# Corleno/Nonstationary_Multivariate_Gaussian_Process

Hardware: AMD Instinct MI355X
Metric: log-posterior evals/sec (N=2048, D=3 nonseparable GP) (higher is better)
Workload: dtype f64

## Files before the change

### nonstationary_multivariate_gaussian_process_amd/csrc/nmgp_api.hip

```cpp
#include <cstdarg>

#include "nmgp_internal.h"

using namespace nmgpk;

enum {
    SC_LOGDET = 0,
    SC_QUAD = 1,
    SC_PRIORQ = 2,
    SC_TRACE = 40,
    SC_OUT = 48,
    SC_MISC = 56,
    SC_COUNT = 128
};

int nmgp_fail(nmgp_ctx* ctx, int code, const char* fmt, ...) {
    char buf[1024];
    va_list ap;
    va_start(ap, fmt);
    vsnprintf(buf, sizeof(buf), fmt, ap);
    va_end(ap);
    if (ctx) ctx->err = buf;
    return code;
}
// ... 774 lines not shown
    return 0;
}

static bool schur_selected(const nmgp_ctx* c, int want_grad) {
    if (want_grad || c->M < 2 || c->svc_schur == 0) return false;
    return true;
}

static int svc_batch_value_schur(nmgp_ctx* c, const double* xs, int xstride, const double* ys, long long ystride, int cps) {
    const int N = c->N, M = c->M, B = c->batch, n1 = (M - 1) * N;
    const long long P = c->P_svc;
    const int xpad = (N + 1) & 1, xoffA = N + 1 + xpad;
    const int ldA = (int)nmgp_ld((size_t)2 * N + 2), ldP = (int)nmgp_ld((size_t)n1 + 1);
    auto r64 = [](size_t v) { return (v + 63) / 64 * 64; };
    const size_t offP = r64((size_t)ldA * N), offPart = r64(offP + (size_t)ldP * n1);
    const size_t need = offPart + (size_t)N * ((N + 255) / 256);
    const size_t bsS = nmgp_ld((size_t)c->n + 1) * (size_t)c->n;
    double* base = c->b_S;
    size_t bsz = bsS;
    if (need > bsS) {
        if (c->b_schur_stride != need) {
            NMGP_TRY(nmgp_dev_alloc(c, &c->b_schur, (size_t)B * need));
            c->b_schur_stride = need;
        }
        base = c->b_schur;
        bsz = need;
    }
    const long long bs = (long long)bsz;
    double* A = base;
    double* Sp = base + offP;
    double* part = base + offPart;
    double* w = c->b_z;
    double* w1 = c->b_z + (size_t)B * N;
    const double* tse = c->b_pars + (P - 1);
    hipStream_t s = c->stream;
    HIP_TRY(c, hipMemsetAsync(c->b_info2, 0, (size_t)B * sizeof(int), s));
    {
        StageScope sp(c, NMGP_STAGE_COV);
        svc_prep(s, c->b_pars, N, M, c->b_ell, c->b_Lv, B);
        int r = svc_schur_build(s, 0, xs, c->b_ell, c->b_Lv, tse, ys, A, ldA, nullptr, nullptr, 0, N, M, B, bs, xstride, ystride, cps);
        if (r) return nmgp_fail(c, r, "unsupported number of outputs M=%d", M);
    }
    {
        StageScope sp(c, NMGP_STAGE_CHOL);
        identity_rows(s, A, ldA, N + 1, N, xpad, B, bs);
        potrf_lower(s, c->stream2, nmgp_chol_events(c, N), A, ldA, N, 1 + xpad, N, c->chol_nb1, c->b_info, B, bs, 1,
                    nmgp_syrk_hook(c));
    }
    {
        StageScope sp(c, NMGP_STAGE_SOLVE);
        get_row(s, A, ldA, N, w, N, B, bs, N);
        tri_gemv_upper(s, A + xoffA, ldA, N, w, c->b_u, part, B, bs, bs);
    }
    {
        StageScope sp(c, NMGP_STAGE_REDUCE);
        chol_logdet_quad(s, A, ldA, N, w, c->b_scal + 2, c->b_scal + 3, B, bs, 16);
    }
    {
        StageScope sp(c, NMGP_STAGE_INVERSE);
        syrk_lower(s, A + xoffA, ldA, A, ldA, N, N, N, B, bs, bs, 2);
    }
    {
        StageScope sp(c, NMGP_STAGE_COV);
        int r = svc_schur_build(s, 1, xs, c->b_ell, c->b_Lv, tse, ys, A, ldA, c->b_u, Sp, ldP, N, M, B, bs, xstride, ystride, cps);
        if (r) return nmgp_fail(c, r, "unsupported number of outputs M=%d", M);
    }
    {
        StageScope sp(c, NMGP_STAGE_CHOL);
        potrf_lower(s, c->stream2, nmgp_chol_events(c, n1), Sp, ldP, n1, 1, 0, c->chol_nb1, c->b_info2, B, bs, 1,
                    nmgp_syrk_hook(c));
    }
    {
        StageScope sp(c, NMGP_STAGE_SOLVE);
        get_row(s, Sp, ldP, n1, w1, n1, B, bs, n1);
    }
    {
        StageScope sp(c, NMGP_STAGE_REDUCE);
        chol_logdet_quad(s, Sp, ldP, n1, w1, c->b_scal + 4, c->b_scal + 5, B, bs, 16);
        svc_schur_combine(s, c->b_Lv, N, M, c->b_scal, 16, c->b_info, c->b_info2, B);
// ... 879 lines not shown
```

### nonstationary_multivariate_gaussian_process_amd/csrc/nmgp_chol.hip

```cpp
#include "nmgp_internal.h"
#include <cstring>

namespace nmgpk {

static inline int cdiv_c(long long a, long long b) { return (int)((a + b - 1) / b); }

typedef double v4d __attribute__((ext_vector_type(4)));

#define SY_BM 128
#define SY_BK 16
#define SY_LD (SY_BM + 16)
#define SY_SB 8

__device__ __forceinline__ int clamp_row_pair(int r, int rows) {
    int rc = r < rows - 1 ? r : rows - 2;
    return rc < 0 ? 0 : rc;
}

__device__ __forceinline__ double fast_recip(double p) {
    double x = __builtin_amdgcn_rcp(p);
    double e = fma(-p, x, 1.0);
    x = fma(x, e, x);
    e = fma(-p, x, 1.0);
    x = fma(x, e, x);
// ... 67 lines not shown
#undef PF
    __syncthreads();
#pragma unroll
    for (int kk = 0; kk < 16; ++kk) {
        const int c = 4 * kk + g;
        if (r < nb && c <= r) A[(size_t)c * lda + r] = a[kk] * rsqrt(pivs[c]);
    }
}

typedef double v2d __attribute__((ext_vector_type(2)));
typedef int v4i __attribute__((ext_vector_type(4)));

__device__ __forceinline__ void syrk_fused_first_block(double* lds, const v4d (&acc)[2][2][2], bool owner, int wj,
                                                       double* __restrict__ C, int ldc, int* __restrict__ info, int goff);

__device__ __forceinline__ void syrk_tile_fast(const double* __restrict__ A, int lda, double* __restrict__ C, int ldc, int K,
                                               int row0, int col0, bool diag, int kt0, bool beta0, int ncw, int yrow,
                                               int nyr, double* sA0, double* sB0, bool skip00 = false,
                                               int* __restrict__ finfo = nullptr, int fgoff = 0, bool mirror = false,
                                               int fresh0 = 0x7fffffff) {
    constexpr int BK = 16;
    constexpr int SBUF = BK * SY_LD;
    const int tid = threadIdx.x, lane = tid & 63, w = tid >> 6;
    const int wi = w & 1, wj = w >> 1;
    const int l15 = lane & 15, l4 = lane >> 4;
    const int rp = tid & 63, cg = tid >> 6;
    const int offA = (cg * lda + row0 + 2 * rp) * 8, offB = (cg * lda + col0 + 2 * rp) * 8;
    const __amdgpu_buffer_rsrc_t rsrc = __builtin_amdgcn_make_buffer_rsrc((void*)A, 0, 0x7fffffff, 0x00020000);
    const int gstep = BK * lda * 8, ghalf = 8 * lda * 8;
    int soff = kt0 * gstep;
    const bool has_y = diag && yrow >= 0;
    const bool ywave = has_y && wi == 0 && wj >= 2;
    const int offY = ((tid & 15) * lda + yrow + (tid >> 4)) * 8;
    double* sY = sB0;
    v4i ra0, ra1, rb0, rb1;
// ... 106 lines not shown
            acc[1][0][1] = __builtin_amdgcn_mfma_f64_16x16x4f64(f1[1], fy, acc[1][0][1], 0, 0, 0);
        }
    };
    for (int kt = kt0; kt < nk; kt += 2) {
        gload();
        if (active) compute(0);
        else if (ywave) compute_y(0, kt * BK);
        sstore(1);
        __syncthreads();
        if (kt + 2 < nk) gload();
        if (active) compute(1);
        else if (ywave) compute_y(1, kt * BK + BK);
        if (kt + 2 < nk) sstore(0);
        __syncthreads();
    }
    if (ywave && l15 < nyr) {
#pragma unroll
        for (int u = 0; u < 2; ++u)
#pragma unroll
            for (int t = 0; t < 2; ++t)
#pragma unroll
                for (int r = 0; r < 4; ++r) {
                    const int j = col0 + 64 * (wj - 2) + 32 * u + 2 * (l4 + 4 * r) + t;
                    C[(size_t)j * ldc + yrow + l15] = -acc[u][0][t][r];
                }
    }
    const bool fowner = finfo != nullptr && wi == 0 && wj < 2;
    if (active && !fowner) {
#pragma unroll
    for (int p = 0; p < 2; ++p)
// ... 23 lines not shown
#pragma unroll
                    for (int r = 0; r < 4; ++r) T[(2 * l15 + sx) * 33 + 2 * (l4 + 4 * r) + tj] = -acc[p][sx][tj][r];
            const int rowm = col0 + wj * 32 + jl;
#pragma unroll
            for (int q = 0; q < 16; ++q) {
                const int il = 2 * q + ih;
                const int colm = row0 + wi * 64 + 32 * p + il;
                const double v = T[il * 33 + jl];
                if (colm > rowm) C[(size_t)colm * ldc + rowm] = v;
            }
        }
    }
    if (finfo != nullptr) syrk_fused_first_block(sA0, acc, fowner, wj, C, ldc, finfo, fgoff);
}

template <int NWJ, int BK>
__device__ __forceinline__ void syrk_tile_body(const double* __restrict__ A, int lda, double* __restrict__ C, int ldc, int mrows,
                                               int ncols, int K, long long bstride, long long cstride, int ktri, int swz,
                                               int nbatch, int bx, int by, int bz0, double* sAb, double* sBb,
                                               int tri_row0 = 0x7fffffff, int tri_k0 = 0, int* __restrict__ finfo = nullptr,
                                               int fistride = 0, int fgoff = 0) {
    const int nyr = (ktri >> 2) & 31;
    const bool skipq = (ktri & 128) != 0;
    const bool mirror = (ktri & 512) != 0;
    const bool rowmajor = (ktri & 1024) != 0;
    const int yrow = nyr ? mrows : -1;
    (void)rowmajor;
    ktri &= 1;
    const int fresh0 = tri_row0 == 0x7fffffff ? 0x7fffffff : tri_row0 + tri_k0;
    constexpr int NT = 128 * NWJ;
    constexpr int CW = 128 / NWJ;
    constexpr int TJ = CW / 16;
    constexpr int NQ = (64 * BK) / NT;
    constexpr int CGS = NT / 64;
    double (*sA)[BK * SY_LD] = reinterpret_cast<double (*)[BK * SY_LD]>(sAb);
    double (*sB)[BK * SY_LD] = reinterpret_cast<double (*)[BK * SY_LD]>(sBb);
// ... 53 lines not shown
            idx -= tri;
            const int blk = idx / (SY_SB * W), in = idx - blk * (SY_SB * W);
            const int base = c0 + W + blk * SY_SB;
            const int rb = gx - base < SY_SB ? gx - base : SY_SB;
            bj = c0 + in / rb;
            bi = base + in % rb;
        }
        }
    }
    if (bi < bj) return;
    bi = __builtin_amdgcn_readfirstlane(bi);
    bj = __builtin_amdgcn_readfirstlane(bj);
    bz = __builtin_amdgcn_readfirstlane(bz);
    A += (size_t)bz * bstride;
    C += (size_t)bz * cstride;
    const bool diag = (bi == bj);
    const int tid = threadIdx.x, lane = tid & 63, w = tid >> 6;
    const int wi = w & 1, wj = w >> 1;
    const int row0 = bi * SY_BM, col0 = bj * SY_BM;
    if constexpr (NWJ == 4 && BK == 16) {
        const int ncw = ncols - col0 >= SY_BM ? SY_BM : ncols - col0;
        if (row0 + SY_BM <= mrows && (ncw == SY_BM || ncw == 64) && col0 + SY_BM <= mrows && (K & 31) == 0 &&
            (long long)(K + 16) * lda * 8 < 0x7fff0000LL) {
            int kt0f = ktri ? row0 / BK : 0;
            if (row0 >= tri_row0) {
                const int z = (row0 - tri_row0 - tri_k0) / BK;
                kt0f = z > 0 ? (z & ~1) : 0;
            }
            syrk_tile_fast(A, lda, C, ldc, K, row0, col0, diag, kt0f, ktri != 0, ncw, yrow, nyr, &sA[0][0], &sB[0][0],
                           skipq && bi == 0 && bj == 0, (finfo != nullptr && bi == 0 && bj == 0) ? finfo + (size_t)bz * fistride : nullptr,
                           fgoff, mirror, fresh0);
            return;
        }
    }
    const int rp = tid & 63, cg = tid >> 6;
    double2 ra[NQ], rb[NQ];

    const int ri = row0 + 2 * rp, rj = col0 + 2 * rp;
    const int ric = clamp_row_pair(ri, mrows), rjc = clamp_row_pair(rj, mrows);
    const bool ix = ri < mrows, iy = ri + 1 < mrows, jx = rj < mrows, jy = rj + 1 < mrows;
    const bool ish = ix && (ric != ri), jsh = jx && (rjc != rj);
    auto gload = [&](int k0) {
#pragma unroll
        for (int q = 0; q < NQ; ++q) {
            const int kc = k0 + cg + CGS * q;
            const double* colp = A + (size_t)(kc < K ? kc : K - 1) * lda;
// ... 69 lines not shown
                for (int tj = 0; tj < TJ; ++tj)
#pragma unroll
                    for (int ti = 0; ti < 4; ++ti)
                        acc[tj][ti] = __builtin_amdgcn_mfma_f64_16x16x4f64(fb[tj], fa[ti], acc[tj][ti], 0, 0, 0);
                if (kk + 1 < BK / 4) {
#pragma unroll
                    for (int t = 0; t < 4; ++t) fa[t] = na[t];
#pragma unroll
                    for (int t = 0; t < TJ; ++t) fb[t] = nb[t];
                }
            }
        }
        if (kt + 1 < nk) sstore(cur ^ 1, (kt + 1) * BK);
        __syncthreads();
    }
    if (active) {
#pragma unroll
        for (int tj = 0; tj < TJ; ++tj)
#pragma unroll
            for (int ti = 0; ti < 4; ++ti)
#pragma unroll
                for (int r = 0; r < 4; ++r) {
                    const int i = row0 + wi * 64 + ti * 16 + (lane & 15);
                    const int j = col0 + wj * CW + tj * 16 + (lane >> 4) + 4 * r;
                    if (i < mrows && j < ncols && i >= j && !(skip00g && i < 64 && j < 64)) C[(size_t)j * ldc + i] = acc[tj][ti][r];
                    if (mirror && i < mrows && j < ncols && i > j) C[(size_t)i * ldc + j] = acc[tj][ti][r];
                }
    }
}

__global__ __launch_bounds__(512, 4) void k_syrk_lower(const double* __restrict__ A, int lda, double* __restrict__ C, int ldc,
                                                        int mrows, int ncols, int K, long long bstride, long long cstride,
                                                        int ktri, int swz, int nbatch, int tri_row0, int tri_k0,
                                                        int* __restrict__ finfo, int fistride, int fgoff) {
    __shared__ __attribute__((aligned(16))) double smem[4 * SY_BK * SY_LD];
    syrk_tile_body<4, SY_BK>(A, lda, C, ldc, mrows, ncols, K, bstride, cstride, ktri, swz, nbatch, blockIdx.x, blockIdx.y,
                             blockIdx.z, smem, smem + 2 * SY_BK * SY_LD, tri_row0, tri_k0, finfo, fistride, fgoff);
}

static thread_local const SyrkHook* g_hook = nullptr;
static int g_syrk_env = 0;
static int g_syrk_yrow = 1;

struct SyrkPlan {
    dim3 grid;
    int swz = 0;
    int kflags = 0;
    int mrows = 0;
    int tiles = 0;
};

static SyrkPlan syrk_plan(int lda, int ldc, int mrows, int ncols, int K, int batch, int ktri, bool compact_only,
// ... 467 lines not shown
    if (g_hook && g_hook->begin) {
        const double elems = (double)ncols * mrows - 0.5 * (double)ncols * (ncols - 1);
        tok = g_hook->begin(g_hook->user, s, 2.0 * K * elems * batch, 8.0 * batch * (2.0 * elems + (double)mrows * K));
    }
    const bool fzb = fuse.info != nullptr && !ktri && cs == bstride && pl.mrows >= SY_BM && (ncols >= SY_BM || ncols == 64) &&
                     (K & 31) == 0 && (long long)(K + 16) * lda * 8 < 0x7fff0000LL;
    SyrkPlan pf = pl;
    if (fzb && pf.swz == 0) {
        pf.grid = dim3((unsigned)((long long)pf.tiles * batch), 1, 1);
        pf.swz = -pf.tiles;
    }
    NMGP_LAUNCH(k_syrk_lower, pf.grid, dim3(512), 0, s, A, lda, C, ldc, pf.mrows, ncols, K, bstride, cs, pf.kflags,
                pf.swz, batch, tri_row0, tri_k0, fzb ? fuse.info : (int*)nullptr, fuse.istride, fuse.goff);
    if (fzb) g_first_block_done = 1;
    if (tok && g_hook->end) g_hook->end(g_hook->user, tok);
}


template <int SRC>
__device__ inline double quad_bcast(double v) {
    constexpr int ctrl = SRC | (SRC << 2) | (SRC << 4) | (SRC << 6);
    int lo = __double2loint(v), hi = __double2hiint(v);
    lo = __builtin_amdgcn_mov_dpp(lo, ctrl, 0xF, 0xF, true);
    hi = __builtin_amdgcn_mov_dpp(hi, ctrl, 0xF, 0xF, true);
    return __hiloint2double(hi, lo);
}

template <int KC, int GC>
__device__ __forceinline__ void trsm_step(double (&x)[16], const double (*Lm)[65], const double* rinv, int g) {
    constexpr int c = 4 * KC + GC;
// ... 935 lines not shown
```

### nonstationary_multivariate_gaussian_process_amd/csrc/nmgp_internal.h

```cpp
#pragma once

#include <hip/hip_runtime.h>
#include <rocblas/rocblas.h>
#include <rocsolver/rocsolver.h>

#include <cmath>
#include <cstdio>
#include <cstdlib>
#include <cstring>
#include <map>
#include <string>
#include <utility>
#include <vector>

#include "nmgp.h"

#define NMGP_JITTER 1e-6
#define NMGP_PRECISION 1e-6

struct DevBuf {
    double* p = nullptr;
    size_t cap = 0;
};

// ... 198 lines not shown
        pending = false;
    }
    ~PriorStreamScope() {
        done();
        join();
    }
};

const SyrkHook* nmgp_syrk_hook(nmgp_ctx* c);

namespace nmgpk {

void svc_prep(hipStream_t s, const double* pars, int N, int M, double* ell, double* Lv, int batch = 1);
int svc_cov_build(hipStream_t s, const double* x, const double* ell, const double* Lv, const double* tse,
                  double* S, int ld, int N, int M, bool full, int batch = 1, long long sstride = 0, int xstride = 0, int cps = 1);
int svc_schur_build(hipStream_t s, int phase, const double* x, const double* ell, const double* Lv, const double* tse,
                    const double* y, double* A, int lda, const double* u, double* S, int ld, int N, int M, int batch,
                    long long bstride, int xstride, long long ystride, int cps);
void svc_schur_combine(hipStream_t s, const double* Lv, int N, int M, double* sc, int sstride, int* info, const int* info2,
                       int batch);
void rbf_cov_sym(hipStream_t s, const double* x, int N, double alpha, double beta, double* out, int ld, bool full,
                 int batch = 1);
void gibbs_cov_sym(hipStream_t s, const double* x, const double* sig, const double* ell, int N, double* out, int ld,
                   bool full);
void pairwise_rect(hipStream_t s, const double* x1, int n1, const double* x2, int n2, int d, double* out);
void rbf_cov_rect(hipStream_t s, const double* x1, int n1, const double* x2, int n2, int d, double alpha, double beta,
                  bool sym, double* out);
void gibbs_cov_rect(hipStream_t s, const double* x1, const double* s1, const double* l1, int n1, const double* x2,
                    const double* s2, const double* l2, int n2, int d, bool sym, double* out);
void kron_product(hipStream_t s, const double* a, int ar, int ac, const double* b, int br, int bc, double* out);
void chol_logdet_quad(hipStream_t s, const double* L, int ld, int n, const double* z, double* out_logdet,
                      double* out_quad, int batch = 1, long long bstride = 0, int ostride = 0);
void col_sumsq(hipStream_t s, const double* R, int ld, int rows, int cols, double* out);
// ... 83 lines not shown
                int ldo, long long bstride);
#define NMGP_SEP_TR_G 128
int sep_traces(hipStream_t s, const double* Cneg, const double* K, const double* alpha, int N, int M, double* out);
void weighted_sum_lower(hipStream_t s, const double* Cneg, const double* wB, int N, int M, double* C);
void sep_prep_b(hipStream_t s, const double* pars, long long P, const double* Y, const double* small, int small_per, int N, int M,
                double* ell, double* sig, double* yt, int B);
void sep_blocks_b(hipStream_t s, const double* x, const double* ell, const double* sig, const double* small, int small_per, int N, int M,
                  double* S, int ldo, long long bstride, double* Kout, int B);
void sep_reduce_b(hipStream_t s, const double* Cneg, const double* K, const double* alpha, const double* small, int small_per, int N,
                  int M, int G, double* C, double* out, double* xi, int B);
void sep_adjoint_b(hipStream_t s, const double* x, const double* ell, const double* sig, const double* U, const double* small,
                   int small_per, int M, const double* C, int N, double* part, double* g, int B);
void two_col_rhs_b(hipStream_t s, const double* pars, long long P, double mu_a, double mu_b, int N, double* R, int B);
void syrk_lower(hipStream_t s, const double* A, int lda, double* C, int ldc, int mrows, int ncols, int K, int batch,
                long long bstride, long long cstride = -1, int ktri = 0, int tri_row0 = 0x7fffffff, int tri_k0 = 0);
void identity_rows(hipStream_t s, double* A, int lda, int row0, int n, int pad, int batch = 1, long long bstride = 0);
void potf2_64(hipStream_t s, double* A, int lda, int nb, int* info, int goff, int batch, long long bstride,
              int istride);
void trsm_64(hipStream_t s, const double* L, int ldl, int nb, double* A, int lda, int rows, int batch,
             long long bstride);
void set_row(hipStream_t s, double* A, int lda, int row, const double* v, int n, int batch, long long bstride,
             long long vstride, int cps = 1);
void get_row(hipStream_t s, const double* A, int lda, int row, double* v, int n, int batch, long long bstride,
             long long vstride);
void potrf_lower(hipStream_t s, hipStream_t s2, hipEvent_t* ev, double* A, int lda, int n, int extra, int xtri,
                 int nb1, int* info, int batch, long long bstride, int istride, const SyrkHook* hook = nullptr,
                 int precise = 0);

bool trtri_post_applies(int n, int xtri, int lda, int batch);
void trtri_upper_post(hipStream_t s, double* S, int ld, int n, int xoff, int batch, long long bs, const SyrkHook* hook);
// ... 3 lines not shown
```

### nonstationary_multivariate_gaussian_process_amd/csrc/nmgp_kernels.hip

```cpp
#include "nmgp_internal.h"
#include <mutex>

namespace nmgpk {

static inline int cdiv(long long a, long long b) { return (int)((a + b - 1) / b); }

__device__ inline double wave_sum(double v) {
#pragma unroll
    for (int off = 32; off > 0; off >>= 1) v += __shfl_down(v, off, 64);
    return v;
}

__device__ inline double block_sum(double v, double* sh ) {
    int lane = threadIdx.x & 63, w = threadIdx.x >> 6;
    v = wave_sum(v);
    __syncthreads();
    if (lane == 0) sh[w] = v;
    __syncthreads();
    int nw = (blockDim.x + 63) >> 6;
    v = (threadIdx.x < nw) ? sh[threadIdx.x] : 0.0;
    if (w == 0) v = wave_sum(v);
    return v;
}

// ... 101 lines not shown
        case 2: launch_svc_cov<2>(s, x, ell, Lv, tse, S, ld, N, full, batch, sstride, xstride, cps); break;
        case 3: launch_svc_cov<3>(s, x, ell, Lv, tse, S, ld, N, full, batch, sstride, xstride, cps); break;
        case 4: launch_svc_cov<4>(s, x, ell, Lv, tse, S, ld, N, full, batch, sstride, xstride, cps); break;
        case 5: launch_svc_cov<5>(s, x, ell, Lv, tse, S, ld, N, full, batch, sstride, xstride, cps); break;
        case 6: launch_svc_cov<6>(s, x, ell, Lv, tse, S, ld, N, full, batch, sstride, xstride, cps); break;
        case 7: launch_svc_cov<7>(s, x, ell, Lv, tse, S, ld, N, full, batch, sstride, xstride, cps); break;
        case 8: launch_svc_cov<8>(s, x, ell, Lv, tse, S, ld, N, full, batch, sstride, xstride, cps); break;
        default: return NMGP_E_UNSUPPORTED;
    }
    return 0;
}

template <int M>
__global__ __launch_bounds__(256) void k_svc_schur_a(const double* __restrict__ x, const double* __restrict__ ell,
                                                      const double* __restrict__ Lv, const double* __restrict__ tse,
                                                      const double* __restrict__ y, double* __restrict__ A, int ld, int N,
                                                      long long astride, int xstride, long long ystride, int cps) {
    constexpr int T = M * (M + 1) / 2;
    constexpr int TJ = 64;
    __shared__ double sx[TJ], sl[TJ];
    const int I = blockIdx.x, J = blockIdx.y;
    if (I < J) return;
    x += (size_t)(blockIdx.z / cps) * xstride;
    y += (size_t)(blockIdx.z / cps) * ystride;
    ell += (size_t)blockIdx.z * N;
    Lv += (size_t)blockIdx.z * N * T;
    tse += (size_t)blockIdx.z * ((size_t)N * (1 + T) + 1);
    A += (size_t)blockIdx.z * astride;
    const int tid = threadIdx.x, lane = tid & 63, w = tid >> 6;
    const int j0 = J * TJ;
    if (tid < TJ) {
        int j = j0 + tid;
        sx[tid] = (j < N) ? x[j] : 0.0;
        sl[tid] = (j < N) ? ell[j] : 1.0;
    }
    __syncthreads();
    const int i = I * 64 + lane;
    if (i >= N) return;
    const double sigma2 = exp(tse[0]);
    const double l00 = Lv[(size_t)i * T];
    const double Ei = sigma2 / (l00 * l00);
    if (J == 0 && w == 0) A[(size_t)i * ld + N] = y[i] / l00;
    const double xi = x[i], li = ell[i];
    const double xi2 = xi * xi, li2 = li * li;
#pragma unroll 2
    for (int jj = 0; jj < TJ / 4; ++jj) {
        const int k = w * (TJ / 4) + jj;
        const int j = j0 + k;
        if (j >= N || j > i) break;
        const double xj = sx[k], lj = sl[k];
        const double dist = (xi2 + xj * xj) - 2.0 * (xi * xj);
        const double Aa = li2 + lj * lj;
        double kv = sqrt(2.0 * (li * lj) / Aa) * exp(-dist / Aa);
        if (i == j) kv = (NMGP_JITTER + kv) + Ei;
        A[(size_t)j * ld + i] = kv;
    }
}

template <int M>
__global__ __launch_bounds__(256) void k_svc_schur_cov(const double* __restrict__ x, const double* __restrict__ ell,
                                                        const double* __restrict__ Lv, const double* __restrict__ tse,
                                                        const double* __restrict__ y, const double* __restrict__ nAinv, int lda,
                                                        const double* __restrict__ u, double* __restrict__ S, int ld, int N,
                                                        long long bstride, int xstride, long long ystride, int cps) {
    constexpr int T = M * (M + 1) / 2;
    constexpr int TJ = 64;
    constexpr int M1 = M - 1;
    __shared__ double sx[TJ], sl[TJ], sL[TJ * T], sg[TJ * M1];
    const int I = blockIdx.x, J = blockIdx.y;
    x += (size_t)(blockIdx.z / cps) * xstride;
    y += (size_t)(blockIdx.z / cps) * ystride;
    ell += (size_t)blockIdx.z * N;
    Lv += (size_t)blockIdx.z * N * T;
    tse += (size_t)blockIdx.z * ((size_t)N * (1 + T) + 1);
    nAinv += (size_t)blockIdx.z * bstride;
    u += (size_t)blockIdx.z * N;
    S += (size_t)blockIdx.z * bstride;
    const int tid = threadIdx.x, lane = tid & 63, w = tid >> 6;
    const int j0 = J * TJ;
    const double sigma2 = exp(tse[0]);
    if (tid < TJ) {
        int j = j0 + tid;
        sx[tid] = (j < N) ? x[j] : 0.0;
        sl[tid] = (j < N) ? ell[j] : 1.0;
    }
    for (int k = tid; k < TJ * T; k += 256) {
        size_t g = (size_t)j0 * T + k;
        sL[k] = (g < (size_t)N * T) ? Lv[g] : 0.0;
    }
    __syncthreads();
    if (tid < TJ) {
        const double l00 = sL[tid * T];
#pragma unroll
        for (int b = 1; b < M; ++b) sg[tid * M1 + b - 1] = sigma2 * sL[tid * T + b * (b + 1) / 2] / (l00 * l00);
    }
    __syncthreads();
    const int i = I * 64 + lane;
    if (i >= N) return;
    const size_t Ns = (size_t)N;
    const int n1 = M1 * N;
    double Li[T];
#pragma unroll
    for (int t = 0; t < T; ++t) Li[t] = Lv[(size_t)i * T + t];
    const double l00 = Li[0];
    const double il2 = 1.0 / (l00 * l00);
    double gi[M1];
#pragma unroll
    for (int a = 1; a < M; ++a) gi[a - 1] = sigma2 * Li[a * (a + 1) / 2] * il2;
    if (J == 0 && w == 0) {
        const double vi = y[i] / l00;
        const double r = vi - (sigma2 * il2) * u[i];
#pragma unroll
        for (int a = 1; a < M; ++a)
            S[((size_t)(a - 1) * Ns + i) * ld + n1] = y[(size_t)a * Ns + i] - Li[a * (a + 1) / 2] * r;
    }
    const double xi = x[i], li = ell[i];
    const double xi2 = xi * xi, li2 = li * li;
#pragma unroll 2
    for (int jj = 0; jj < TJ / 4; ++jj) {
        const int k = w * (TJ / 4) + jj;
        const int j = j0 + k;
        if (j >= N) break;
        const double xj = sx[k], lj = sl[k];
        const double dist = (xi2 + xj * xj) - 2.0 * (xi * xj);
        const double Aa = li2 + lj * lj;
        double kv = sqrt(2.0 * (li * lj) / Aa) * exp(-dist / Aa);
        if (i == j) kv = NMGP_JITTER + kv;
        const double nai = nAinv[(size_t)j * lda + i];
#pragma unroll
        for (int a = 1; a < M; ++a) {
#pragma unroll
            for (int b = 1; b <= a; ++b) {
                if (b == a && i < j) continue;
                double s = 0.0;
#pragma unroll
                for (int c = 1; c <= b; ++c) s += Li[a * (a + 1) / 2 + c] * sL[k * T + b * (b + 1) / 2 + c];
                double v = kv * s;
                if (i == j) v += sigma2 * ((a == b ? 1.0 : 0.0) + Li[a * (a + 1) / 2] * Li[b * (b + 1) / 2] * il2);
                v += gi[a - 1] * nai * sg[k * M1 + b - 1];
                S[((size_t)(b - 1) * Ns + j) * ld + ((size_t)(a - 1) * Ns + i)] = v;
            }
        }
    }
}

template <int M>
static void launch_svc_schur(hipStream_t s, const double* x, const double* ell, const double* Lv, const double* tse,
                             const double* y, double* A, int lda, const double* u, double* S, int ld, int N, int batch,
                             long long bstride, int xstride, long long ystride, int cps, int phase) {
    dim3 grid(cdiv(N, 64), cdiv(N, 64), batch);
    if (phase == 0)
        NMGP_LAUNCH((k_svc_schur_a<M>), grid, dim3(256), 0, s, x, ell, Lv, tse, y, A, lda, N, bstride, xstride, ystride, cps);
    else
        NMGP_LAUNCH((k_svc_schur_cov<M>), grid, dim3(256), 0, s, x, ell, Lv, tse, y, A, lda, u, S, ld, N, bstride, xstride,
                    ystride, cps);
}

int svc_schur_build(hipStream_t s, int phase, const double* x, const double* ell, const double* Lv, const double* tse,
                    const double* y, double* A, int lda, const double* u, double* S, int ld, int N, int M, int batch,
                    long long bstride, int xstride, long long ystride, int cps) {
    if (cps < 1) cps = 1;
    switch (M) {
        case 2: launch_svc_schur<2>(s, x, ell, Lv, tse, y, A, lda, u, S, ld, N, batch, bstride, xstride, ystride, cps, phase); break;
        case 3: launch_svc_schur<3>(s, x, ell, Lv, tse, y, A, lda, u, S, ld, N, batch, bstride, xstride, ystride, cps, phase); break;
        case 4: launch_svc_schur<4>(s, x, ell, Lv, tse, y, A, lda, u, S, ld, N, batch, bstride, xstride, ystride, cps, phase); break;
        case 5: launch_svc_schur<5>(s, x, ell, Lv, tse, y, A, lda, u, S, ld, N, batch, bstride, xstride, ystride, cps, phase); break;
        case 6: launch_svc_schur<6>(s, x, ell, Lv, tse, y, A, lda, u, S, ld, N, batch, bstride, xstride, ystride, cps, phase); break;
        case 7: launch_svc_schur<7>(s, x, ell, Lv, tse, y, A, lda, u, S, ld, N, batch, bstride, xstride, ystride, cps, phase); break;
        case 8: launch_svc_schur<8>(s, x, ell, Lv, tse, y, A, lda, u, S, ld, N, batch, bstride, xstride, ystride, cps, phase); break;
        default: return NMGP_E_UNSUPPORTED;
    }
    return 0;
}

__global__ __launch_bounds__(256) void k_svc_schur_combine(const double* __restrict__ Lv, int N, int T, double* __restrict__ sc,
                                                            int sstride, int* __restrict__ info, const int* __restrict__ info2) {
    __shared__ double sh[16];
    Lv += (size_t)blockIdx.x * N * T;
    sc += (size_t)blockIdx.x * sstride;
    double a = 0.0;
    for (int i = threadIdx.x; i < N; i += blockDim.x) a += log(Lv[(size_t)i * T]);
    a = block_sum(a, sh);
    if (threadIdx.x == 0) {
        sc[0] = (2.0 * a + sc[2]) + sc[4];
// ... 849 lines not shown
```

Measured before the change: 1636.

## Fuse Schur covariance build into SYRK epilogue and fold identity rows into build

The separate kernel that rebuilt the Schur-complement covariance from the stored A^{-1} product is replaced by an epilogue inside the SYRK tile kernel. The kernel now writes the M-1 output blocks directly from the register accumulators through an LDS patch, with a per-tile table of per-point scalars. This removes the write and re-read of the N x N inverse-product matrix and one launch. The first-phase build now also writes the identity/pad rows and computes two rows per thread with paired stores, over a triangular tile enumeration. In exchange the SYRK kernel gets heavier epilogue register and LDS pressure, and its scattered stores to S may be poorly coalesced.

```diff
diff --git a/nonstationary_multivariate_gaussian_process_amd/csrc/nmgp_api.hip b/nonstationary_multivariate_gaussian_process_amd/csrc/nmgp_api.hip
--- a/nonstationary_multivariate_gaussian_process_amd/csrc/nmgp_api.hip
+++ b/nonstationary_multivariate_gaussian_process_amd/csrc/nmgp_api.hip
@@ -812,7 +812,7 @@
     const int ldA = (int)nmgp_ld((size_t)2 * N + 2), ldP = (int)nmgp_ld((size_t)n1 + 1);
     auto r64 = [](size_t v) { return (v + 63) / 64 * 64; };
     const size_t offP = r64((size_t)ldA * N), offPart = r64(offP + (size_t)ldP * n1);
-    const size_t need = offPart + (size_t)N * ((N + 255) / 256);
+    const size_t need = r64(offPart + (size_t)N * ((N + 255) / 256));
     const size_t bsS = nmgp_ld((size_t)c->n + 1) * (size_t)c->n;
     double* base = c->b_S;
     size_t bsz = bsS;
@@ -836,12 +836,11 @@
     {
         StageScope sp(c, NMGP_STAGE_COV);
         svc_prep(s, c->b_pars, N, M, c->b_ell, c->b_Lv, B);
-        int r = svc_schur_build(s, 0, xs, c->b_ell, c->b_Lv, tse, ys, A, ldA, nullptr, nullptr, 0, N, M, B, bs, xstride, ystride, cps);
+        int r = svc_schur_a(s, xs, c->b_ell, c->b_Lv, tse, ys, A, ldA, xpad, N, M, B, bs, xstride, ystride, cps);
         if (r) return nmgp_fail(c, r, "unsupported number of outputs M=%d", M);
     }
     {
         StageScope sp(c, NMGP_STAGE_CHOL);
-        identity_rows(s, A, ldA, N + 1, N, xpad, B, bs);
         potrf_lower(s, c->stream2, nmgp_chol_events(c, N), A, ldA, N, 1 + xpad, N, c->chol_nb1, c->b_info, B, bs, 1,
                     nmgp_syrk_hook(c));
     }
@@ -856,11 +855,8 @@
     }
     {
         StageScope sp(c, NMGP_STAGE_INVERSE);
-        syrk_lower(s, A + xoffA, ldA, A, ldA, N, N, N, B, bs, bs, 2);
-    }
-    {
-        StageScope sp(c, NMGP_STAGE_COV);
-        int r = svc_schur_build(s, 1, xs, c->b_ell, c->b_Lv, tse, ys, A, ldA, c->b_u, Sp, ldP, N, M, B, bs, xstride, ystride, cps);
+        const SchurEpi e{xs, c->b_ell, c->b_Lv, tse, ys, c->b_u, Sp, ldP, N, xstride, cps, ystride, bs};
+        int r = syrk_schur(s, A + xoffA, ldA, N, M, B, e);
         if (r) return nmgp_fail(c, r, "unsupported number of outputs M=%d", M);
     }
     {
diff --git a/nonstationary_multivariate_gaussian_process_amd/csrc/nmgp_chol.hip b/nonstationary_multivariate_gaussian_process_amd/csrc/nmgp_chol.hip
--- a/nonstationary_multivariate_gaussian_process_amd/csrc/nmgp_chol.hip
+++ b/nonstationary_multivariate_gaussian_process_amd/csrc/nmgp_chol.hip
@@ -105,11 +105,143 @@
 __device__ __forceinline__ void syrk_fused_first_block(double* lds, const v4d (&acc)[2][2][2], bool owner, int wj,
                                                        double* __restrict__ C, int ldc, int* __restrict__ info, int goff);
 
+#define SY_SMEM (4 * SY_BK * SY_LD)
+#define SCHUR_PATCH (32 * 33)
+#define SY_SCHUR_SMEM (8 * SCHUR_PATCH + 6 * 256)
+static_assert(SY_SCHUR_SMEM >= SY_SMEM && SY_SCHUR_SMEM * 8 * 2 <= 160 * 1024, "Schur epilogue LDS");
+
+template <int M>
+__device__ __forceinline__ double svc_schur_value(double sigma2, int a, int b, bool rc, const double* __restrict__ Lr, double il2,
+                                                  const double* __restrict__ Lc, double kv, double nai, double gcb) {
+    constexpr int UR = M <= 3 ? 8 : 1;
+    const double gra = sigma2 * Lr[a * (a + 1) / 2] * il2;
+    double s = 0.0;
+#pragma unroll UR
+    for (int q = 1; q <= b; ++q) s += Lr[a * (a + 1) / 2 + q] * Lc[b * (b + 1) / 2 + q];
+    double v = kv * s;
+    if (rc) v += sigma2 * ((a == b ? 1.0 : 0.0) + Lr[a * (a + 1) / 2] * Lr[b * (b + 1) / 2] * il2);
+    v += gra * nai * gcb;
+    return v;
+}
+
+template <int M, bool ALLB>
+__device__ __forceinline__ void svc_schur_entries(const SchurEpi& e, double sigma2, int r, const double* __restrict__ Lr, double il2,
+                                                  int c, double kv, double nai, const double* gc) {
+    constexpr int T = M * (M + 1) / 2;
+    constexpr int UR = M <= 3 ? 8 : 1;
+    const size_t Ns = (size_t)e.N;
+    const double* __restrict__ Lc = e.Lv + (size_t)c * T;
+    const double lcc = M <= 4 ? 0.0 : Lc[0];
+#pragma unroll UR
+    for (int a = 1; a < M; ++a) {
+#pragma unroll UR
+        for (int b = 1; b <= (ALLB ? a : a - 1); ++b) {
+            const double gcb = M <= 4 ? gc[b - 1] : sigma2 * Lc[b * (b + 1) / 2] / (lcc * lcc);
+            e.S[((size_t)(b - 1) * Ns + c) * e.ld + ((size_t)(a - 1) * Ns + r)] =
+                svc_schur_value<M>(sigma2, a, b, r == c, Lr, il2, Lc, kv, nai, gcb);
+        }
+    }
+}
+
+constexpr int svc_gstride(int M) { return M + 2; }
+
+template <int M>
+__device__ __forceinline__ void svc_schur_gtable(const SchurEpi& e, double* lds, int row0, int col0, int tid) {
+    constexpr int T = M * (M + 1) / 2, GS = svc_gstride(M);
+    if constexpr (M <= 4) {
+        double* gt = lds + 8 * SCHUR_PATCH;
+        if (tid < 256) {
+            const int loc = tid < 128 ? col0 + tid : row0 + tid - 128;
+            if (loc < e.N) {
+                const double sigma2 = exp(e.tse[0]);
+                const double* Lc = e.Lv + (size_t)loc * T;
+                const double l00 = Lc[0];
+#pragma unroll
+                for (int b = 1; b < M; ++b) gt[tid * GS + b - 1] = sigma2 * Lc[b * (b + 1) / 2] / (l00 * l00);
+                gt[tid * GS + M - 1] = 1.0 / (l00 * l00);
+                gt[tid * GS + M] = e.x[loc];
+                gt[tid * GS + M + 1] = e.ell[loc];
+            }
+        }
+        __syncthreads();
+    }
+}
+
+template <int M>
+__device__ __forceinline__ void svc_schur_patch(const SchurEpi& e, double* P, const double* lds, int i0, int j0, int row0, int col0,
+                                                int lane) {
+    constexpr int T_ = M * (M + 1) / 2, GS = svc_gstride(M);
+    constexpr int QU = M <= 3 ? 2 : 1;
+    const int N = e.N;
+    const size_t Ns = (size_t)N;
+    const double sigma2 = exp(e.tse[0]);
+    const double* gt = lds + 8 * SCHUR_PATCH;
+    const int lo = lane & 31, hi = lane >> 5;
+    __builtin_amdgcn_wave_barrier();
+#pragma unroll
+    for (int pass = 0; pass < 2; ++pass) {
+        if (pass == 1 && M == 2) break;
+        const int r = (pass == 0 ? i0 : j0) + lo;
+        if (r < N) {
+            const double* __restrict__ Lr = e.Lv + (size_t)r * T_;
+            const double xr = e.x[r], lr = e.ell[r];
+            const double xr2 = xr * xr, lr2 = lr * lr;
+            const double l00 = Lr[0];
+            const double il2 = 1.0 / (l00 * l00);
+#pragma unroll QU
+            for (int q = 0; q < 16; ++q) {
+                const int o = 2 * q + hi;
+                const int il = pass == 0 ? lo : o, jl = pass == 0 ? o : lo;
+                const int c = (pass == 0 ? j0 : i0) + o;
+                if (pass == 0 ? (c > r || c >= N) : (c <= r || c >= N)) continue;
+                const double* gc = gt + (pass == 0 ? c - col0 : 128 + c - row0) * GS;
+                if (pass == 1 && M == 3) {
+                    e.S[(size_t)c * e.ld + (Ns + r)] = P[il * 33 + jl];
+                    continue;
+                }
+                const double xc = M <= 4 ? gc[M] : e.x[c], lc = M <= 4 ? gc[M + 1] : e.ell[c];
+                const double dist = (xr2 + xc * xc) - 2.0 * (xr * xc);
+                const double Aa = lr2 + lc * lc;
+                double kv = sqrt(2.0 * (lr * lc) / Aa) * exp(-dist / Aa);
+                if (r == c) kv = NMGP_JITTER + kv;
+                const double nai = P[il * 33 + jl];
+                if (pass == 0) {
+                    svc_schur_entries<M, true>(e, sigma2, r, Lr, il2, c, kv, nai, gc);
+                    if (M == 3 && c < r) {
+                        const double* Lc = e.Lv + (size_t)c * T_;
+                        P[il * 33 + jl] = svc_schur_value<M>(sigma2, 2, 1, false, Lc, gc[M - 1], Lr, kv, nai, gt[(128 + r - row0) * GS]);
+                    }
+                } else {
+                    svc_schur_entries<M, false>(e, sigma2, r, Lr, il2, c, kv, nai, gc);
+                }
+            }
+        }
+        __builtin_amdgcn_wave_barrier();
+    }
+}
+
+template <int M>
+__device__ __forceinline__ void svc_schur_yrow(const SchurEpi& e, int i) {
+    constexpr int T = M * (M + 1) / 2;
+    if (i >= e.N) return;
+    const size_t Ns = (size_t)e.N;
+    const int n1 = (M - 1) * e.N;
+    const double sigma2 = exp(e.tse[0]);
+    const double* Li = e.Lv + (size_t)i * T;
+    const double l00 = Li[0];
+    const double il2 = 1.0 / (l00 * l00);
+    const double vi = e.y[i] / l00;
+    const double r = vi - (sigma2 * il2) * e.u[i];
+#pragma unroll
+    for (int a = 1; a < M; ++a) e.S[((size_t)(a - 1) * Ns + i) * e.ld + n1] = e.y[(size_t)a * Ns + i] - Li[a * (a + 1) / 2] * r;
+}
+
+template <int SM = 0>
 __device__ __forceinline__ void syrk_tile_fast(const double* __restrict__ A, int lda, double* __restrict__ C, int ldc, int K,
                                                int row0, int col0, bool diag, int kt0, bool beta0, int ncw, int yrow,
                                                int nyr, double* sA0, double* sB0, bool skip00 = false,
                                                int* __restrict__ finfo = nullptr, int fgoff = 0, bool mirror = false,
-                                               int fresh0 = 0x7fffffff) {
+                                               int fresh0 = 0x7fffffff, const SchurEpi* se = nullptr) {
     constexpr int BK = 16;
     constexpr int SBUF = BK * SY_LD;
     const int tid = threadIdx.x, lane = tid & 63, w = tid >> 6;
@@ -246,6 +378,24 @@
         if (kt + 2 < nk) sstore(0);
         __syncthreads();
     }
+    if constexpr (SM > 0) {
+        svc_schur_gtable<SM>(*se, sA0, row0, col0, tid);
+        if (active) {
+            double* P = sA0 + w * SCHUR_PATCH;
+#pragma unroll
+            for (int p = 0; p < 2; ++p) {
+#pragma unroll
+                for (int sx = 0; sx < 2; ++sx)
+#pragma unroll
+                    for (int tj = 0; tj < 2; ++tj)
+#pragma unroll
+                        for (int r = 0; r < 4; ++r) P[(2 * l15 + sx) * 33 + 2 * (l4 + 4 * r) + tj] = -acc[p][sx][tj][r];
+                svc_schur_patch<SM>(*se, P, sA0, row0 + wi * 64 + 32 * p, col0 + wj * 32, row0, col0, lane);
+            }
+        }
+        if (diag && wj == 0) svc_schur_yrow<SM>(*se, row0 + wi * 64 + lane);
+        return;
+    }
     if (ywave && l15 < nyr) {
 #pragma unroll
         for (int u = 0; u < 2; ++u)
@@ -299,12 +449,12 @@
     if (finfo != nullptr) syrk_fused_first_block(sA0, acc, fowner, wj, C, ldc, finfo, fgoff);
 }
 
-template <int NWJ, int BK>
+template <int NWJ, int BK, int SM = 0>
 __device__ __forceinline__ void syrk_tile_body(const double* __restrict__ A, int lda, double* __restrict__ C, int ldc, int mrows,
                                                int ncols, int K, long long bstride, long long cstride, int ktri, int swz,
                                                int nbatch, int bx, int by, int bz0, double* sAb, double* sBb,
                                                int tri_row0 = 0x7fffffff, int tri_k0 = 0, int* __restrict__ finfo = nullptr,
-                                               int fistride = 0, int fgoff = 0) {
+                                               int fistride = 0, int fgoff = 0, const SchurEpi* sep = nullptr) {
     const int nyr = (ktri >> 2) & 31;
     const bool skipq = (ktri & 128) != 0;
     const bool mirror = (ktri & 512) != 0;
@@ -388,6 +538,19 @@
     bz = __builtin_amdgcn_readfirstlane(bz);
     A += (size_t)bz * bstride;
     C += (size_t)bz * cstride;
+    SchurEpi se{};
+    if constexpr (SM > 0) {
+        static_assert(NWJ == 4 && BK == 16, "the Schur epilogue assumes 8 waves of 64 x 32");
+        constexpr int T = SM * (SM + 1) / 2;
+        se = *sep;
+        se.x += (size_t)(bz / se.cps) * se.xstride;
+        se.y += (size_t)(bz / se.cps) * se.ystride;
+        se.ell += (size_t)bz * se.N;
+        se.Lv += (size_t)bz * se.N * T;
+        se.tse += (size_t)bz * ((size_t)se.N * (1 + T) + 1);
+        se.u += (size_t)bz * se.N;
+        se.S += (size_t)bz * se.bstride;
+    }
     const bool diag = (bi == bj);
     const int tid = threadIdx.x, lane = tid & 63, w = tid >> 6;
     const int wi = w & 1, wj = w >> 1;
@@ -401,9 +564,9 @@
                 const int z = (row0 - tri_row0 - tri_k0) / BK;
                 kt0f = z > 0 ? (z & ~1) : 0;
             }
-            syrk_tile_fast(A, lda, C, ldc, K, row0, col0, diag, kt0f, ktri != 0, ncw, yrow, nyr, &sA[0][0], &sB[0][0],
-                           skipq && bi == 0 && bj == 0, (finfo != nullptr && bi == 0 && bj == 0) ? finfo + (size_t)bz * fistride : nullptr,
-                           fgoff, mirror, fresh0);
+            syrk_tile_fast<SM>(A, lda, C, ldc, K, row0, col0, diag, kt0f, ktri != 0, ncw, yrow, nyr, &sA[0][0], &sB[0][0],
+                               skipq && bi == 0 && bj == 0, (finfo != nullptr && bi == 0 && bj == 0) ? finfo + (size_t)bz * fistride : nullptr,
+                               fgoff, mirror, fresh0, &se);
             return;
         }
     }
@@ -503,6 +666,25 @@
         if (kt + 1 < nk) sstore(cur ^ 1, (kt + 1) * BK);
         __syncthreads();
     }
+    if constexpr (SM > 0) {
+        svc_schur_gtable<SM>(se, sAb, row0, col0, tid);
+        if (active) {
+            double* P = sAb + w * SCHUR_PATCH;
+#pragma unroll
+            for (int h = 0; h < 2; ++h) {
+#pragma unroll
+                for (int tj = 0; tj < TJ; ++tj)
+#pragma unroll
+                    for (int t2 = 0; t2 < 2; ++t2)
+#pragma unroll
+                        for (int r = 0; r < 4; ++r)
+                            P[(t2 * 16 + (lane & 15)) * 33 + tj * 16 + (lane >> 4) + 4 * r] = acc[tj][2 * h + t2][r];
+                svc_schur_patch<SM>(se, P, sAb, row0 + wi * 64 + 32 * h, col0 + wj * CW, row0, col0, lane);
+            }
+        }
+        if (diag && wj == 0) svc_schur_yrow<SM>(se, row0 + wi * 64 + lane);
+        return;
+    }
     if (active) {
 #pragma unroll
         for (int tj = 0; tj < TJ; ++tj)
@@ -525,6 +707,14 @@
     __shared__ __attribute__((aligned(16))) double smem[4 * SY_BK * SY_LD];
     syrk_tile_body<4, SY_BK>(A, lda, C, ldc, mrows, ncols, K, bstride, cstride, ktri, swz, nbatch, blockIdx.x, blockIdx.y,
                              blockIdx.z, smem, smem + 2 * SY_BK * SY_LD, tri_row0, tri_k0, finfo, fistride, fgoff);
+}
+
+template <int M>
+__global__ __launch_bounds__(512, 4) void k_syrk_schur(const double* __restrict__ A, int lda, int N, long long bstride, int kflags,
+                                                        int swz, int nbatch, SchurEpi se) {
+    __shared__ __attribute__((aligned(16))) double smem[SY_SCHUR_SMEM];
+    syrk_tile_body<4, SY_BK, M>(A, lda, nullptr, 0, N, N, N, bstride, 0, kflags, swz, nbatch, blockIdx.x, blockIdx.y, blockIdx.z,
+                                smem, smem + 2 * SY_BK * SY_LD, 0x7fffffff, 0, nullptr, 0, 0, &se);
 }
 
 static thread_local const SyrkHook* g_hook = nullptr;
@@ -1022,6 +1212,26 @@
                 pf.swz, batch, tri_row0, tri_k0, fzb ? fuse.info : (int*)nullptr, fuse.istride, fuse.goff);
     if (fzb) g_first_block_done = 1;
     if (tok && g_hook->end) g_hook->end(g_hook->user, tok);
+}
+
+int syrk_schur(hipStream_t s, const double* X, int lda, int N, int M, int batch, const SchurEpi& e) {
+    if (N <= 0) return 0;
+    if (M < 2 || M > 8) return NMGP_E_UNSUPPORTED;
+    const SyrkPlan pl = syrk_plan(lda, lda, N, N, N, batch, 2, false);
+    void* tok = nullptr;
+    if (g_hook && g_hook->begin) {
+        const double elems = (double)N * N - 0.5 * (double)N * (N - 1);
+        const double n1 = (double)(M - 1) * N;
+        tok = g_hook->begin(g_hook->user, s, 2.0 * N * elems * batch, 8.0 * batch * ((double)N * N + 0.5 * n1 * (n1 + 1) + n1));
+    }
+    switch (M) {
+#define SCHUR_CASE(m) \
+        case m: NMGP_LAUNCH(k_syrk_schur<m>, pl.grid, dim3(512), 0, s, X, lda, pl.mrows, e.bstride, pl.kflags, pl.swz, batch, e); break;
+        SCHUR_CASE(2) SCHUR_CASE(3) SCHUR_CASE(4) SCHUR_CASE(5) SCHUR_CASE(6) SCHUR_CASE(7) SCHUR_CASE(8)
+#undef SCHUR_CASE
+    }
+    if (tok && g_hook->end) g_hook->end(g_hook->user, tok);
+    return 0;
 }
 
 
diff --git a/nonstationary_multivariate_gaussian_process_amd/csrc/nmgp_internal.h b/nonstationary_multivariate_gaussian_process_amd/csrc/nmgp_internal.h
--- a/nonstationary_multivariate_gaussian_process_amd/csrc/nmgp_internal.h
+++ b/nonstationary_multivariate_gaussian_process_amd/csrc/nmgp_internal.h
@@ -236,9 +236,8 @@
 void svc_prep(hipStream_t s, const double* pars, int N, int M, double* ell, double* Lv, int batch = 1);
 int svc_cov_build(hipStream_t s, const double* x, const double* ell, const double* Lv, const double* tse,
                   double* S, int ld, int N, int M, bool full, int batch = 1, long long sstride = 0, int xstride = 0, int cps = 1);
-int svc_schur_build(hipStream_t s, int phase, const double* x, const double* ell, const double* Lv, const double* tse,
-                    const double* y, double* A, int lda, const double* u, double* S, int ld, int N, int M, int batch,
-                    long long bstride, int xstride, long long ystride, int cps);
+int svc_schur_a(hipStream_t s, const double* x, const double* ell, const double* Lv, const double* tse, const double* y, double* A,
+                int lda, int pad, int N, int M, int batch, long long bstride, int xstride, long long ystride, int cps);
 void svc_schur_combine(hipStream_t s, const double* Lv, int N, int M, double* sc, int sstride, int* info, const int* info2,
                        int batch);
 void rbf_cov_sym(hipStream_t s, const double* x, int N, double alpha, double beta, double* out, int ld, bool full,
@@ -352,6 +351,22 @@
 void two_col_rhs_b(hipStream_t s, const double* pars, long long P, double mu_a, double mu_b, int N, double* R, int B);
 void syrk_lower(hipStream_t s, const double* A, int lda, double* C, int ldc, int mrows, int ncols, int K, int batch,
                 long long bstride, long long cstride = -1, int ktri = 0, int tri_row0 = 0x7fffffff, int tri_k0 = 0);
+struct SchurEpi {
+    const double* x;
+    const double* ell;
+    const double* Lv;
+    const double* tse;
+    const double* y;
+    const double* u;
+    double* S;
+    int ld;
+    int N;
+    int xstride;
+    int cps;
+    long long ystride;
+    long long bstride;
+};
+int syrk_schur(hipStream_t s, const double* X, int lda, int N, int M, int batch, const SchurEpi& e);
 void identity_rows(hipStream_t s, double* A, int lda, int row0, int n, int pad, int batch = 1, long long bstride = 0);
 void potf2_64(hipStream_t s, double* A, int lda, int nb, int* info, int goff, int batch, long long bstride,
               int istride);
diff --git a/nonstationary_multivariate_gaussian_process_amd/csrc/nmgp_kernels.hip b/nonstationary_multivariate_gaussian_process_amd/csrc/nmgp_kernels.hip
--- a/nonstationary_multivariate_gaussian_process_amd/csrc/nmgp_kernels.hip
+++ b/nonstationary_multivariate_gaussian_process_amd/csrc/nmgp_kernels.hip
@@ -139,13 +139,23 @@
 template <int M>
 __global__ __launch_bounds__(256) void k_svc_schur_a(const double* __restrict__ x, const double* __restrict__ ell,
                                                       const double* __restrict__ Lv, const double* __restrict__ tse,
-                                                      const double* __restrict__ y, double* __restrict__ A, int ld, int N,
+                                                      const double* __restrict__ y, double* __restrict__ A, int ld, int pad, int N,
                                                       long long astride, int xstride, long long ystride, int cps) {
     constexpr int T = M * (M + 1) / 2;
-    constexpr int TJ = 64;
+    constexpr int TJ = 32, TI = 128;
+    constexpr int BAND = 64 * (NMGP_XTRI_SEED_BLOCKS + 1);
     __shared__ double sx[TJ], sl[TJ];
-    const int I = blockIdx.x, J = blockIdx.y;
-    if (I < J) return;
+    const int NI = (N + TI - 1) / TI, NJ = (N + TJ - 1) / TJ;
+    int ntl = 0;
+    for (int J = 0; J < NJ; ++J) ntl += NI - J / 4 + 1;
+    const int per = (ntl + 7) / 8;
+    const int g = blockIdx.x, t = (g & 7) * per + (g >> 3);
+    if ((g >> 3) >= per || t >= ntl) return;
+    int rem = t, J = 0;
+    while (rem >= NI - J / 4 + 1) {
+        rem -= NI - J / 4 + 1;
+        ++J;
+    }
     x += (size_t)(blockIdx.z / cps) * xstride;
     y += (size_t)(blockIdx.z / cps) * ystride;
     ell += (size_t)blockIdx.z * N;
@@ -154,145 +164,88 @@
     A += (size_t)blockIdx.z * astride;
     const int tid = threadIdx.x, lane = tid & 63, w = tid >> 6;
     const int j0 = J * TJ;
+    if (rem == NI - J / 4) {
+        const int row0 = N + 1 + pad;
+        for (int k = 0; k < TJ / 4; ++k) {
+            const int c = j0 + w * (TJ / 4) + k;
+            if (c >= N) break;
+            const int rb = c / 64 * 64;
+            const int nq = 1 + pad + ((rb + BAND < N ? rb + BAND : N) - rb);
+            double* col = A + (size_t)c * ld;
+            for (int q = lane; q < nq; q += 64) {
+                const int r = q <= pad ? N + q : row0 + rb + (q - 1 - pad);
+                double v = 0.0;
+                if (q == 0) v = y[c] / Lv[(size_t)c * T];
+                else if (r == row0 + c) v = 1.0;
+                col[r] = v;
+            }
+        }
+        return;
+    }
+    const int I = J / 4 + rem;
     if (tid < TJ) {
-        int j = j0 + tid;
+        const int j = j0 + tid;
         sx[tid] = (j < N) ? x[j] : 0.0;
         sl[tid] = (j < N) ? ell[j] : 1.0;
     }
     __syncthreads();
-    const int i = I * 64 + lane;
+    const int i = I * TI + 2 * lane;
     if (i >= N) return;
+    const bool two = i + 1 < N;
     const double sigma2 = exp(tse[0]);
-    const double l00 = Lv[(size_t)i * T];
-    const double Ei = sigma2 / (l00 * l00);
-    if (J == 0 && w == 0) A[(size_t)i * ld + N] = y[i] / l00;
-    const double xi = x[i], li = ell[i];
-    const double xi2 = xi * xi, li2 = li * li;
-#pragma unroll 2
+    double xi[2], li[2], xi2[2], li2[2], Ei[2];
+#pragma unroll
+    for (int h = 0; h < 2; ++h) {
+        const int ih = two ? i + h : i;
+        const double l00 = Lv[(size_t)ih * T];
+        Ei[h] = sigma2 / (l00 * l00);
+        xi[h] = x[ih];
+        li[h] = ell[ih];
+        xi2[h] = xi[h] * xi[h];
+        li2[h] = li[h] * li[h];
+    }
     for (int jj = 0; jj < TJ / 4; ++jj) {
         const int k = w * (TJ / 4) + jj;
         const int j = j0 + k;
-        if (j >= N || j > i) break;
+        if (j >= N || j > i + 1) break;
         const double xj = sx[k], lj = sl[k];
-        const double dist = (xi2 + xj * xj) - 2.0 * (xi * xj);
-        const double Aa = li2 + lj * lj;
-        double kv = sqrt(2.0 * (li * lj) / Aa) * exp(-dist / Aa);
-        if (i == j) kv = (NMGP_JITTER + kv) + Ei;
-        A[(size_t)j * ld + i] = kv;
+        double kv[2];
+#pragma unroll
+        for (int h = 0; h < 2; ++h) {
+            const double dist = (xi2[h] + xj * xj) - 2.0 * (xi[h] * xj);
+            const double Aa = li2[h] + lj * lj;
+            kv[h] = sqrt(2.0 * (li[h] * lj) / Aa) * exp(-dist / Aa);
+            if (i + h == j) kv[h] = (NMGP_JITTER + kv[h]) + Ei[h];
+        }
+        double* dst = A + (size_t)j * ld + i;
+        if (two && j <= i) *reinterpret_cast<double2*>(dst) = make_double2(kv[0], kv[1]);
+        else if (two) dst[1] = kv[1];
+        else dst[0] = kv[0];
     }
 }
 
 template <int M>
-__global__ __launch_bounds__(256) void k_svc_schur_cov(const double* __restrict__ x, const double* __restrict__ ell,
-                                                        const double* __restrict__ Lv, const double* __restrict__ tse,
-                                                        const double* __restrict__ y, const double* __restrict__ nAinv, int lda,
-                                                        const double* __restrict__ u, double* __restrict__ S, int ld, int N,
-                                                        long long bstride, int xstride, long long ystride, int cps) {
-    constexpr int T = M * (M + 1) / 2;
-    constexpr int TJ = 64;
-    constexpr int M1 = M - 1;
-    __shared__ double sx[TJ], sl[TJ], sL[TJ * T], sg[TJ * M1];
-    const int I = blockIdx.x, J = blockIdx.y;
-    x += (size_t)(blockIdx.z / cps) * xstride;
-    y += (size_t)(blockIdx.z / cps) * ystride;
-    ell += (size_t)blockIdx.z * N;
-    Lv += (size_t)blockIdx.z * N * T;
-    tse += (size_t)blockIdx.z * ((size_t)N * (1 + T) + 1);
-    nAinv += (size_t)blockIdx.z * bstride;
-    u += (size_t)blockIdx.z * N;
-    S += (size_t)blockIdx.z * bstride;
-    const int tid = threadIdx.x, lane = tid & 63, w = tid >> 6;
-    const int j0 = J * TJ;
-    const double sigma2 = exp(tse[0]);
-    if (tid < TJ) {
-        int j = j0 + tid;
-        sx[tid] = (j < N) ? x[j] : 0.0;
-        sl[tid] = (j < N) ? ell[j] : 1.0;
-    }
-    for (int k = tid; k < TJ * T; k += 256) {
-        size_t g = (size_t)j0 * T + k;
-        sL[k] = (g < (size_t)N * T) ? Lv[g] : 0.0;
-    }
-    __syncthreads();
-    if (tid < TJ) {
-        const double l00 = sL[tid * T];
-#pragma unroll
-        for (int b = 1; b < M; ++b) sg[tid * M1 + b - 1] = sigma2 * sL[tid * T + b * (b + 1) / 2] / (l00 * l00);
-    }
-    __syncthreads();
-    const int i = I * 64 + lane;
-    if (i >= N) return;
-    const size_t Ns = (size_t)N;
-    const int n1 = M1 * N;
-    double Li[T];
-#pragma unroll
-    for (int t = 0; t < T; ++t) Li[t] = Lv[(size_t)i * T + t];
-    const double l00 = Li[0];
-    const double il2 = 1.0 / (l00 * l00);
-    double gi[M1];
-#pragma unroll
-    for (int a = 1; a < M; ++a) gi[a - 1] = sigma2 * Li[a * (a + 1) / 2] * il2;
-    if (J == 0 && w == 0) {
-        const double vi = y[i] / l00;
-        const double r = vi - (sigma2 * il2) * u[i];
-#pragma unroll
-        for (int a = 1; a < M; ++a)
-            S[((size_t)(a - 1) * Ns + i) * ld + n1] = y[(size_t)a * Ns + i] - Li[a * (a + 1) / 2] * r;
-    }
-    const double xi = x[i], li = ell[i];
-    const double xi2 = xi * xi, li2 = li * li;
-#pragma unroll 2
-    for (int jj = 0; jj < TJ / 4; ++jj) {
-        const int k = w * (TJ / 4) + jj;
-        const int j = j0 + k;
-        if (j >= N) break;
-        const double xj = sx[k], lj = sl[k];
-        const double dist = (xi2 + xj * xj) - 2.0 * (xi * xj);
-        const double Aa = li2 + lj * lj;
-        double kv = sqrt(2.0 * (li * lj) / Aa) * exp(-dist / Aa);
-        if (i == j) kv = NMGP_JITTER + kv;
-        const double nai = nAinv[(size_t)j * lda + i];
-#pragma unroll
-        for (int a = 1; a < M; ++a) {
-#pragma unroll
-            for (int b = 1; b <= a; ++b) {
-                if (b == a && i < j) continue;
-                double s = 0.0;
-#pragma unroll
-                for (int c = 1; c <= b; ++c) s += Li[a * (a + 1) / 2 + c] * sL[k * T + b * (b + 1) / 2 + c];
-                double v = kv * s;
-                if (i == j) v += sigma2 * ((a == b ? 1.0 : 0.0) + Li[a * (a + 1) / 2] * Li[b * (b + 1) / 2] * il2);
-                v += gi[a - 1] * nai * sg[k * M1 + b - 1];
-                S[((size_t)(b - 1) * Ns + j) * ld + ((size_t)(a - 1) * Ns + i)] = v;
-            }
-        }
-    }
-}
-
-template <int M>
-static void launch_svc_schur(hipStream_t s, const double* x, const double* ell, const double* Lv, const double* tse,
-                             const double* y, double* A, int lda, const double* u, double* S, int ld, int N, int batch,
-                             long long bstride, int xstride, long long ystride, int cps, int phase) {
-    dim3 grid(cdiv(N, 64), cdiv(N, 64), batch);
-    if (phase == 0)
-        NMGP_LAUNCH((k_svc_schur_a<M>), grid, dim3(256), 0, s, x, ell, Lv, tse, y, A, lda, N, bstride, xstride, ystride, cps);
-    else
-        NMGP_LAUNCH((k_svc_schur_cov<M>), grid, dim3(256), 0, s, x, ell, Lv, tse, y, A, lda, u, S, ld, N, bstride, xstride,
-                    ystride, cps);
-}
-
-int svc_schur_build(hipStream_t s, int phase, const double* x, const double* ell, const double* Lv, const double* tse,
-                    const double* y, double* A, int lda, const double* u, double* S, int ld, int N, int M, int batch,
-                    long long bstride, int xstride, long long ystride, int cps) {
+static void launch_svc_schur_a(hipStream_t s, const double* x, const double* ell, const double* Lv, const double* tse,
+                               const double* y, double* A, int lda, int pad, int N, int batch, long long bstride, int xstride,
+                               long long ystride, int cps) {
+    const int NI = cdiv(N, 128), NJ = cdiv(N, 32);
+    int ntl = 0;
+    for (int J = 0; J < NJ; ++J) ntl += NI - J / 4 + 1;
+    NMGP_LAUNCH((k_svc_schur_a<M>), dim3(8 * cdiv(ntl, 8), 1, batch), dim3(256), 0, s, x, ell, Lv, tse, y, A, lda, pad, N, bstride,
+                xstride, ystride, cps);
+}
+
+int svc_schur_a(hipStream_t s, const double* x, const double* ell, const double* Lv, const double* tse, const double* y, double* A,
+                int lda, int pad, int N, int M, int batch, long long bstride, int xstride, long long ystride, int cps) {
     if (cps < 1) cps = 1;
     switch (M) {
-        case 2: launch_svc_schur<2>(s, x, ell, Lv, tse, y, A, lda, u, S, ld, N, batch, bstride, xstride, ystride, cps, phase); break;
-        case 3: launch_svc_schur<3>(s, x, ell, Lv, tse, y, A, lda, u, S, ld, N, batch, bstride, xstride, ystride, cps, phase); break;
-        case 4: launch_svc_schur<4>(s, x, ell, Lv, tse, y, A, lda, u, S, ld, N, batch, bstride, xstride, ystride, cps, phase); break;
-        case 5: launch_svc_schur<5>(s, x, ell, Lv, tse, y, A, lda, u, S, ld, N, batch, bstride, xstride, ystride, cps, phase); break;
-        case 6: launch_svc_schur<6>(s, x, ell, Lv, tse, y, A, lda, u, S, ld, N, batch, bstride, xstride, ystride, cps, phase); break;
-        case 7: launch_svc_schur<7>(s, x, ell, Lv, tse, y, A, lda, u, S, ld, N, batch, bstride, xstride, ystride, cps, phase); break;
-        case 8: launch_svc_schur<8>(s, x, ell, Lv, tse, y, A, lda, u, S, ld, N, batch, bstride, xstride, ystride, cps, phase); break;
+        case 2: launch_svc_schur_a<2>(s, x, ell, Lv, tse, y, A, lda, pad, N, batch, bstride, xstride, ystride, cps); break;
+        case 3: launch_svc_schur_a<3>(s, x, ell, Lv, tse, y, A, lda, pad, N, batch, bstride, xstride, ystride, cps); break;
+        case 4: launch_svc_schur_a<4>(s, x, ell, Lv, tse, y, A, lda, pad, N, batch, bstride, xstride, ystride, cps); break;
+        case 5: launch_svc_schur_a<5>(s, x, ell, Lv, tse, y, A, lda, pad, N, batch, bstride, xstride, ystride, cps); break;
+        case 6: launch_svc_schur_a<6>(s, x, ell, Lv, tse, y, A, lda, pad, N, batch, bstride, xstride, ystride, cps); break;
+        case 7: launch_svc_schur_a<7>(s, x, ell, Lv, tse, y, A, lda, pad, N, batch, bstride, xstride, ystride, cps); break;
+        case 8: launch_svc_schur_a<8>(s, x, ell, Lv, tse, y, A, lda, pad, N, batch, bstride, xstride, ystride, cps); break;
         default: return NMGP_E_UNSUPPORTED;
     }
     return 0;
```

Measured after the change: 1694, median of 6. 1.04x the previous value.
